# prashantpandeygit/solvingpapers

Hardware: AMD Instinct MI355X
Metric: training tokens/sec, LLaMA3-8B-shape bf16 (higher is better)
Workload: dtype bf16; 1 GPU; model=llama3_8b, global_batch=4, seq_len=8192, parallelism=dp1, micro_batch=1, grad_accum=4, params=8030261248

## Files before the change

csrc/include/attn_params.h:

```cpp
#pragma once
#include "attn_common.h"

#define SPA_DBG_BRH(b, r, R, h, H) (SPA_DBG_OK(b, p.B) & SPA_DBG_OK(r, R) & SPA_DBG_OK(h, H))

namespace spa {

struct AttnParams {
  const bf16* q; const bf16* k; const bf16* v; const bf16* o; const bf16* dout;
  bf16* out; bf16* dq; bf16* dk; bf16* dv;
  float* lse; const float* lse_in; float* delta; float* dqacc;
  int B, H, Hkv, Tq, Tk;
  long sqb, sqt, sqh, skb, skt, skh, svb, svt, svh, sob, sot, soh;
  long sdob, sdot, sdoh;
  long sdqb, sdqt, sdqh, sdkb, sdkt, sdkh, sdvb, sdvt, sdvh;
  float scale;
  float scale_log2;
  int causal_off;
  int hsplit;
  float* dkacc; float* dvacc;
  unsigned seed_lo, seed_hi, drop_thr;
  float drop_scale;
  const int64_t* seed_ptr;
  long long* stamp;
  int xcd;
  bf16* dsbuf;
  long ds_kvstride;
  int ds_nqt, ds_nkt;
  int ksplit;
  float* part;
  float* mlpart;
  int part_ld;
  int vhalf;
  float* rowk;
  int rowk_ld;
};

void launch_dkdv5(AttnParams& p, bool causal, hipStream_t st);
void launch_bwd_short(AttnParams& p, bool causal, hipStream_t st);

__device__ __forceinline__ long ds_index(int qt, int kt, int g, int G, int nkt, bool causal) {
  const int qb = qt >> 1, t = qt & 1;
  const long step = causal ? (long)qb * (qb + 1) + kt : (long)qb * nkt + kt;
  return (step * G + g) * 2 + t;
}
inline long ds_kv_elems(int nq64, int nkt, int G, bool causal) {
  return 1024L * 2 * G * (causal ? (long)nq64 * (nq64 + 1) : (long)nq64 * nkt);
}
__device__ __forceinline__ int ds_slot(int s, int h, int k) { return (k >> 2) * 16 + (2 * s + h) * 4 + (k & 3); }

template <int HD, int NDT = HD / 32>
__device__ __forceinline__ void store_kv_grad(const AttnParams& p, const f32x16 (&acc)[NDT], bool is_k,
                                              int b, int hk, int key, int split, int hh, int dt0 = 0) {
  if (key >= p.Tk) return;
  if (!(SPA_DBG_BRH(b, key, p.Tk, hk, p.Hkv) & SPA_DBG_OK(split, p.hsplit))) return;
  static_assert(NDT <= HD / 32, "store_kv_grad: more tiles than the head dim");
  constexpr int DT = NDT;
  if (p.hsplit == 1) {
    bf16* dst = (is_k ? p.dk + b * p.sdkb + (long)key * p.sdkt + hk * p.sdkh
                      : p.dv + b * p.sdvb + (long)key * p.sdvt + hk * p.sdvh) + 32 * dt0;
    const float sc = is_k ? p.scale : 1.f;
#pragma unroll
    for (int dt = 0; dt < DT; ++dt)
#pragma unroll
      for (int g = 0; g < 4; ++g) {
        bf16x4 w;
#pragma unroll
        for (int i = 0; i < 4; ++i) w[i] = (bf16)(acc[dt][4 * g + i] * sc);
        *reinterpret_cast<bf16x4*>(dst + 32 * dt + 8 * g + 4 * hh) = w;
      }
  } else {
    float* dst = (is_k ? p.dkacc : p.dvacc) +
                 ((((long)split * p.B + b) * p.Tk + key) * p.Hkv + hk) * HD + 32 * dt0;
#pragma unroll
    for (int dt = 0; dt < DT; ++dt)
#pragma unroll
      for (int g = 0; g < 4; ++g) {
        f32x4 w;
#pragma unroll
        for (int i = 0; i < 4; ++i) w[i] = acc[dt][4 * g + i];
        *reinterpret_cast<f32x4*>(dst + 32 * dt + 8 * g + 4 * hh) = w;
      }
  }
}


}
```

csrc/kernels/attention.hip:

```cpp
#include "attn_common.h"
#include "attn_params.h"

SPA_DEBUG_TU("attention.hip")

namespace spa {



__device__ __forceinline__ unsigned mix32(unsigned x) {
  x ^= x >> 16; x *= 0x7feb352dU; x ^= x >> 15; x *= 0x846ca68bU; x ^= x >> 16;
  return x;
}
__device__ __forceinline__ unsigned drop_base(const AttnParams& p, int b, int h) {
  unsigned lo = p.seed_lo, hi = p.seed_hi;
  if (p.seed_ptr) {
    const uint64_t sd = (uint64_t)*p.seed_ptr;
    lo = (unsigned)(sd & 0xffffffffu);
    hi = (unsigned)(sd >> 32);
  }
  return mix32(lo ^ mix32(hi + (unsigned)(b * p.H + h) * 0x9E3779B9U));
}
__device__ __forceinline__ bool drop_keep(unsigned base, int q, int key, unsigned thr) {
  return (mix32(base + (unsigned)q * 0x85EBCA6BU + (unsigned)key * 0xC2B2AE35U) >> 8) >= thr;
}
// ... 1258 lines not shown
      dso[ab] = 8 * ds_slot(g, pp & 1, key) + 4 * (pp >> 1);
    }
  }
  f32x16 acc[2][DT];
#pragma unroll
  for (int t = 0; t < 2; ++t)
#pragma unroll
    for (int i = 0; i < DT; ++i) acc[t][i] = splat16(0.f);

  auto compute = [&](int j, const bf16* sl) {
    if (j >= nsteps_w) return;
    const bf16* Ks = sl;
    const bf16* Dw = sl + KIMG + wave * WSLOT;
    const bool l0 = live(2 * qb, j), l1 = live(2 * qb + 1, j);
#pragma unroll
    for (int s = 0; s < 2; ++s) {
      bf16x8 kt[DT];
#pragma unroll
      for (int dt = 0; dt < DT; ++dt) kt[dt] = ld_tr(Ks + 16 * s * HD, off.tra[dt], off.trb[dt]);
      const bf16x8 d0 = ld_tr(Dw + 512 * s, dso[0], dso[1]);
      const bf16x8 d1 = ld_tr(Dw + 1024 + 512 * s, dso[0], dso[1]);
      if (l0) {
#pragma unroll
        for (int dt = 0; dt < DT; ++dt) acc[0][dt] = mfma32(kt[dt], d0, acc[0][dt]);
      }
      if (l1) {
#pragma unroll
        for (int dt = 0; dt < DT; ++dt) acc[1][dt] = mfma32(kt[dt], d1, acc[1][dt]);
      }
    }
  };
  if (nsteps > 0) issue(0, 0);
  if (nsteps > 1) issue(1, 1);
  for (int j = 0; j < nsteps; j += 3) {
#pragma unroll
    for (int r = 0; r < 3; ++r) {
      const int jj = j + r;
      if (jj < nsteps) {
        if (jj + 1 < nsteps) asm volatile("s_waitcnt vmcnt(6)" ::: "memory");
        else asm volatile("s_waitcnt vmcnt(0)" ::: "memory");
        asm volatile("s_waitcnt lgkmcnt(0)" ::: "memory");
        __builtin_amdgcn_s_barrier();
        if (jj + 2 < nsteps) issue(jj + 2, (r + 2) % 3);
        compute(jj, smem + r * SLOT);
      }
    }
  }
  if (!uvalid) return;
#pragma unroll
  for (int t = 0; t < 2; ++t) {
    const int q = qb * 64 + 32 * t + (lane & 31);
    if (q >= p.Tq || !SPA_DBG_BRH(b, q, p.Tq, h, p.H)) continue;
    bf16* op = p.dq + b * p.sdqb + (long)q * p.sdqt + h * p.sdqh;
#pragma unroll
    for (int dt = 0; dt < DT; ++dt)
#pragma unroll
      for (int g = 0; g < 4; ++g) {
        bf16x4 wv;
#pragma unroll
        for (int i = 0; i < 4; ++i) wv[i] = (bf16)(acc[t][dt][4 * g + i] * p.scale);
        *reinterpret_cast<bf16x4*>(op + 32 * dt + 8 * g + 4 * hh) = wv;
      }
  }
}

template <int HDK, bool CAUSAL, bool NT>
__global__ __launch_bounds__(256, 2) void attn_bwd_dq_ds256_kernel(AttnParams p) {
  static_assert(HDK == 256 || HDK == 192, "dq_ds256: q/k head dim 192 or 256");
  constexpr int HD = 256, DT = HDK / 32, KIMG = 32 * HD, WSLOT = 1024, SLOT = KIMG + 4 * WSLOT, NSLOT = 3;
  __shared__ __attribute__((aligned(16))) bf16 smem[NSLOT * SLOT];
  const int tid = threadIdx.x, lane = tid & 63;
  const int wave = __builtin_amdgcn_readfirstlane(tid >> 6);
  const int hh = lane >> 5;
  const int G = p.H / p.Hkv;
  const int nqt = cdiv(p.Tq, 32);
  const int upkv = nqt * G;
  const int wgpkv = cdiv(upkv, 4);
  const int nbkv = p.B * p.Hkv;
  const int bkv = blockIdx.x % nbkv;
  const int w = CAUSAL ? wgpkv - 1 - (int)(blockIdx.x / nbkv) : (int)(blockIdx.x / nbkv);
  const int b = bkv / p.Hkv, hk = bkv % p.Hkv;
  SPA_DBG_CHECK(b, p.B);
  const int u = 4 * w + wave;
  const bool uvalid = u < upkv;
  const int qt = uvalid ? u / G : 0;
  const int h = hk * G + (uvalid ? u % G : 0);
  auto unit_steps = [&](int uu) {
    const int qtt = uu / G;
    return CAUSAL ? cdiv(min(p.Tk, qtt * 32 + 32 + p.causal_off), 32) : cdiv(p.Tk, 32);
  };
  const int nsteps_w = uvalid ? unit_steps(u) : 0;
  const int nsteps = unit_steps(min(4 * w + 3, upkv - 1));

  const bf16* kbase = p.k + b * p.skb + hk * p.skh;
  unsigned kvo[4];
#pragma unroll
  for (int j = 0; j < 4; ++j) {
    const int r = 8 * wave + 2 * j + (lane >> 5);
    kvo[j] = (unsigned)(((long)r * p.skt + 8 * ((lane & 31) ^ swz<HD>(r))) * 2);
  }
  const bf16* dskv = p.dsbuf + ((long)b * p.Hkv + hk) * p.ds_kvstride;
  const int g = h - hk * G;
  auto live = [&](int kt) { return uvalid && qt < p.ds_nqt && (!CAUSAL || kt <= qt); };
  auto issue = [&](int j, int slot) {
    bf16* sl = smem + slot * SLOT;
    const int key0 = 32 * j;
// ... 342 lines not shown
        }
      } else {
        if (causal) attn_fwd_kernel<HDK_, HDV_, NW, true, false><<<gx, NW * 64, 0, st>>>(p);
        else attn_fwd_kernel<HDK_, HDV_, NW, false, false><<<gx, NW * 64, 0, st>>>(p);
      }
    });
  }
  if (p.ksplit > 1) {
    const long n = (long)B * H * Tq * (HDV / 8);
    HDKV_SWITCH(HDK, HDV, { attn_fwd_merge_kernel<HDV_><<<(int)cdiv(n, 256L), 256, 0, st>>>(p); });
  }
  SPA_LAUNCH_CHECK();
  return {out, lse};
}

template <int HDK, int HDV, bool DROP>
static void launch_bwd(AttnParams& p, bool causal, bool fused, int dkdv_mode, int nkv, hipStream_t st,
                       const at::TensorOptions& bf16_opts) {
  constexpr int NW = dq_waves<HDK, HDV>();
  constexpr int MT = (HDK <= 128 && HDV <= 128) ? 2 : 1;
  constexpr bool PAIRED_OK = HDK == HDV && HDK <= 128 && !DROP;
  const int g2 = nkv * p.hsplit;
  if constexpr (HDK == HDV && HDK <= 128 && !DROP) {
    if (fused) {
      const long rows = (long)p.B * p.Tq * p.H;
      attn_delta_kernel<HDK><<<(int)cdiv(rows, 256 / (HDK / 8)), 256, 0, st>>>(p);
      if (causal) attn_bwd_dkdv_kernel<HDK, HDV, true, MT, true, false><<<g2, 256, 0, st>>>(p);
      else attn_bwd_dkdv_kernel<HDK, HDV, false, MT, true, false><<<g2, 256, 0, st>>>(p);
      const long n = rows * (HDK / 8);
      attn_dq_store_kernel<HDK><<<(int)std::min<long>((n + 255) / 256, 65536), 256, 0, st>>>(p);
      return;
    }
  }
  if constexpr (HDK == 128 && HDV == 128 && !DROP) {
    const char* de = getenv("SPA_ATTN_DQ_DS");
    const bool want = !(de && atoi(de) == 0);
    const long kv_bytes = 2 * ds_kv_elems(cdiv(p.Tq, 64), cdiv(p.Tk, 32), p.H / p.Hkv, causal);
    if (want && p.hsplit == 1 && p.Tk > 0 && dkdv_mode == 0 && (!causal || p.causal_off == 0) &&
        kv_bytes < 0x7fffffffL) {
      const long rows = (long)p.B * p.Tq * p.H;
      const char* v5e = getenv("SPA_ATTN_DKDV5");
      const bool v5 = !(v5e && atoi(v5e) == 0);
      if (!v5) attn_delta_kernel<HDK><<<(int)cdiv(rows, 256 / (HDK / 8)), 256, 0, st>>>(p);
      p.ds_nqt = cdiv(p.Tq, 32);
      p.ds_nkt = cdiv(p.Tk, 32);
      p.ds_kvstride = ds_kv_elems(cdiv(p.Tq, 64), p.ds_nkt, p.H / p.Hkv, causal);
      at::Tensor dsb = at::empty({(long)p.B * p.Hkv * p.ds_kvstride}, bf16_opts);
      p.dsbuf = (bf16*)dsb.data_ptr();
      at::Tensor rowk;
      if (v5) {
        p.rowk_ld = cdiv(p.Tq, 64) * 64;
        rowk = at::empty({(long)p.B * p.H * 2 * p.rowk_ld}, bf16_opts.dtype(at::kFloat));
        p.rowk = rowk.data_ptr<float>();
        launch_dkdv5(p, causal, st);
      } else if (causal) attn_bwd_dkdv3_kernel<HDK, HDV, true, true><<<nkv, 512, 0, st>>>(p);
      else attn_bwd_dkdv3_kernel<HDK, HDV, false, true><<<nkv, 512, 0, st>>>(p);
      const int G = p.H / p.Hkv;
      const int wg = cdiv(cdiv(p.Tq, 64) * G, 4) * p.B * p.Hkv;
      const char* ne = getenv("SPA_ATTN_DS_NT");
      const bool nt = !(ne && atoi(ne) == 0);
      if (nt) {
        if (causal) attn_bwd_dq_ds_kernel<HDK, true, true><<<wg, 256, 0, st>>>(p);
        else attn_bwd_dq_ds_kernel<HDK, false, true><<<wg, 256, 0, st>>>(p);
      } else {
        if (causal) attn_bwd_dq_ds_kernel<HDK, true, false><<<wg, 256, 0, st>>>(p);
        else attn_bwd_dq_ds_kernel<HDK, false, false><<<wg, 256, 0, st>>>(p);
      }
      return;
    }
  }
  if constexpr (((HDK == 256 && HDV == 256) || (HDK == 192 && HDV == 128)) && !DROP) {
    const char* de = getenv("SPA_ATTN_DQ_DS");
    const int dsm = de ? atoi(de) : 1;
    const bool want = dsm != 0;
    const int G = p.H / p.Hkv;
    const long kv_bytes = 2 * ds_kv_elems(cdiv(p.Tq, 64), cdiv(p.Tk, 32), G, causal);
    const int wg = cdiv(cdiv(p.Tq, 32) * G, 4) * p.B * p.Hkv;
    if (want && (wg >= 512 || dsm == 2) && p.Tk > 0 && dkdv_mode == 0 && (!causal || p.causal_off == 0) &&
        kv_bytes < 0x7fffffffL) {
      const long rows = (long)p.B * p.Tq * p.H;
      attn_delta_kernel<HDV><<<(int)cdiv(rows, 256 / (HDV / 8)), 256, 0, st>>>(p);
      p.ds_nqt = cdiv(p.Tq, 32);
      p.ds_nkt = cdiv(p.Tk, 32);
      p.ds_kvstride = ds_kv_elems(cdiv(p.Tq, 64), p.ds_nkt, G, causal);
      at::Tensor dsb = at::empty({(long)p.B * p.Hkv * p.ds_kvstride}, bf16_opts);
      p.dsbuf = (bf16*)dsb.data_ptr();
      const int g2 = nkv * p.hsplit;
      bool paired_mla = false, dvs = false;
      AttnParams pk = p;
      at::Tensor dkpart;
      if constexpr (HDK == 256 && HDV == 256) {
        const char* ve = getenv("SPA_ATTN_DKDV256");
        dvs = !(ve && atoi(ve) == 0) && G % p.hsplit == 0;
        if (dvs) {
          if (causal) attn_bwd_dkdv3_kernel<HDK, HDV, true, true, true><<<g2, 512, 0, st>>>(p);
          else attn_bwd_dkdv3_kernel<HDK, HDV, false, true, true><<<g2, 512, 0, st>>>(p);
          int hs2 = p.hsplit;
          while (nkv * hs2 < 1024 && hs2 < G) {
            int d = hs2 + 1;
            while (G % d) ++d;
            hs2 = d;
          }
          pk.hsplit = hs2;
          if (hs2 > 1) {
            dkpart = at::empty({(long)hs2 * p.B * p.Tk * p.Hkv * HDK}, bf16_opts.dtype(at::kFloat));
            pk.dkacc = dkpart.data_ptr<float>();
// ... 19 lines not shown
      if (nt) {
        if (causal) attn_bwd_dq_ds256_kernel<HDK, true, true><<<wg, 256, 0, st>>>(p);
        else attn_bwd_dq_ds256_kernel<HDK, false, true><<<wg, 256, 0, st>>>(p);
      } else {
        if (causal) attn_bwd_dq_ds256_kernel<HDK, true, false><<<wg, 256, 0, st>>>(p);
        else attn_bwd_dq_ds256_kernel<HDK, false, false><<<wg, 256, 0, st>>>(p);
      }
      const long kr = (long)p.B * p.Tk * p.Hkv;
      if ((dvs ? pk : p).hsplit > 1)
        attn_kv_reduce_kernel<HDK><<<(int)std::min<long>((kr * (HDK / 8) + 255) / 256, 65536), 256, 0, st>>>(dvs ? pk : p, 1);
      if (p.hsplit > 1)
        attn_kv_reduce_kernel<HDV><<<(int)std::min<long>((kr * (HDV / 8) + 255) / 256, 65536), 256, 0, st>>>(p, 0);
      return;
    }
  }
  const int grid = cdiv(p.Tq, 32 * NW) * p.H * p.B;
  p.ksplit = p.Tk > 0 ? attn_ksplit(grid, cdiv(p.Tk, attn_bn<HDK, HDV>())) : 1;
  at::Tensor dqpart;
  if (p.ksplit > 1) {
    dqpart = at::empty({(long)p.ksplit * p.B * p.Tq * p.H * HDK}, bf16_opts.dtype(at::kFloat));
    p.part = dqpart.data_ptr<float>();
    p.part_ld = HDK;
  }
  if (causal) attn_bwd_dq_kernel<HDK, HDV, NW, true, DROP><<<grid * p.ksplit, NW * 64, 0, st>>>(p);
  else attn_bwd_dq_kernel<HDK, HDV, NW, false, DROP><<<grid * p.ksplit, NW * 64, 0, st>>>(p);
  if (p.ksplit > 1) {
    const long n = (long)p.B * p.Tq * p.H * (HDK / 8);
    attn_dq_reduce_kernel<HDK><<<(int)cdiv(n, 256L), 256, 0, st>>>(p);
  }
  if (p.Tk == 0) return;
  const bool piped = PAIRED_OK && (dkdv_mode == 3 || (dkdv_mode == 0 && HDV == 128));
  if (piped) {
    if constexpr (PAIRED_OK) {
      if (causal) attn_bwd_dkdv3_kernel<HDK, HDV, true><<<g2, 512, 0, st>>>(p);
      else attn_bwd_dkdv3_kernel<HDK, HDV, false><<<g2, 512, 0, st>>>(p);
    }
  } else {
    if (causal) attn_bwd_dkdv_kernel<HDK, HDV, true, MT, false, DROP><<<g2, 256, 0, st>>>(p);
    else attn_bwd_dkdv_kernel<HDK, HDV, false, MT, false, DROP><<<g2, 256, 0, st>>>(p);
  }
  if (p.hsplit > 1) {
    const long rows = (long)p.B * p.Tk * p.Hkv;
    attn_kv_reduce_kernel<HDK><<<(int)std::min<long>((rows * (HDK / 8) + 255) / 256, 65536), 256, 0, st>>>(p, 1);
    attn_kv_reduce_kernel<HDV><<<(int)std::min<long>((rows * (HDV / 8) + 255) / 256, 65536), 256, 0, st>>>(p, 0);
  }
}

static at::Tensor& last_stamps() {
  static at::Tensor t;
  return t;
}
at::Tensor attn_bwd_stamps() { return last_stamps().defined() ? last_stamps().view({-1, 8}).clone() : at::Tensor(); }

void attn_bwd(const at::Tensor& dout, const at::Tensor& q, const at::Tensor& k, const at::Tensor& v,
              const at::Tensor& out, const at::Tensor& lse, const at::Tensor& dq, const at::Tensor& dk,
              const at::Tensor& dv, double scale, bool causal, double dropout_p, int64_t seed,
              const c10::optional<at::Tensor>& seed_t) {
  check_qkv(dout, "dout"); check_qkv(q, "q"); check_qkv(k, "k"); check_qkv(v, "v"); check_qkv(out, "out");
  check_qkv(dq, "dq"); check_qkv(dk, "dk"); check_qkv(dv, "dv");
  const int B = q.size(0), Tq = q.size(1), H = q.size(2), HDK = q.size(3), HDV = v.size(3);
  const int Tk = k.size(1), Hkv = k.size(2);
  TORCH_CHECK(lse.is_contiguous() && lse.numel() == (int64_t)B * H * Tq);
  TORCH_CHECK(dq.sizes() == q.sizes() && dk.sizes() == k.sizes() && dv.sizes() == v.sizes());
  TORCH_CHECK(dout.sizes() == out.sizes() && out.size(3) == HDV && out.size(2) == H && out.size(1) == Tq);
  const bool drop = dropout_p > 0.0;
  TORCH_CHECK(!drop || HDK == HDV, "attn: dropout needs equal q/k and v head dims");
  DeviceGuard g(q.device());
  auto delta = at::empty({B, H, Tq}, q.options().dtype(at::kFloat));
  AttnParams p{};
  p.q = (const bf16*)q.data_ptr(); p.k = (const bf16*)k.data_ptr(); p.v = (const bf16*)v.data_ptr();
  p.o = (const bf16*)out.data_ptr(); p.dout = (const bf16*)dout.data_ptr();
  p.dq = (bf16*)dq.data_ptr(); p.dk = (bf16*)dk.data_ptr(); p.dv = (bf16*)dv.data_ptr();
  p.lse_in = lse.data_ptr<float>(); p.delta = delta.data_ptr<float>();
  p.B = B; p.H = H; p.Hkv = Hkv; p.Tq = Tq; p.Tk = Tk;
  fill_strides(p, q, k, v);
  fill_dropout(p, dropout_p, seed, seed_t);
  p.sob = out.stride(0); p.sot = out.stride(1); p.soh = out.stride(2);
  p.sdob = dout.stride(0); p.sdot = dout.stride(1); p.sdoh = dout.stride(2);
  p.sdqb = dq.stride(0); p.sdqt = dq.stride(1); p.sdqh = dq.stride(2);
  p.sdkb = dk.stride(0); p.sdkt = dk.stride(1); p.sdkh = dk.stride(2);
  p.sdvb = dv.stride(0); p.sdvt = dv.stride(1); p.sdvh = dv.stride(2);
  p.scale = (float)scale; p.scale_log2 = (float)(scale * 1.4426950408889634);
  p.causal_off = Tk - Tq;
  p.xcd = xcd_order(B, Hkv);
  p.ksplit = 1;
  if (B * H == 0) return;
  auto st = stream();
  if (Tq == 0) { dk.zero_(); dv.zero_(); return; }
  static const bool want_fused = getenv("SPA_ATTN_BWD_FUSED") && atoi(getenv("SPA_ATTN_BWD_FUSED")) != 0;
  const bool fused = want_fused && Tk > 0 && HDK <= 128 && HDK == HDV && !drop;
  const char* sse = getenv("SPA_ATTN_SHORT");
  const bool want_short = !(sse && atoi(sse) == 0);
  if (want_short && !fused && !drop && HDK == 64 && HDV == 64 && H == Hkv && Tq <= 256 && Tk <= 256) {
    launch_bwd_short(p, causal, st);
    SPA_LAUNCH_CHECK();
    return;
  }
  at::Tensor dqacc;
  if (fused) {
    dqacc = at::zeros({B, Tq, H, HDK}, q.options().dtype(at::kFloat));
    p.dqacc = dqacc.data_ptr<float>();
  }
  const int dkdv_mode = getenv("SPA_ATTN_DKDV") ? atoi(getenv("SPA_ATTN_DKDV")) : 0;
  const int G = H / Hkv;
  const int nkv = cdiv(Tk, 128) * Hkv * B;
  int hsplit = 1;
  const char* kbe = getenv("SPA_ATTN_KVBLOCKS");
  const int kvblocks = kbe ? std::max(1, atoi(kbe)) : 512;
  if (!fused)
    while (nkv * hsplit < kvblocks && hsplit < G) {
      int d = hsplit + 1;
      while (G % d) ++d;
      hsplit = d;
    }
  const bool pairedk = HDK == HDV && HDK <= 128 && !drop && (dkdv_mode == 3 || (dkdv_mode == 0 && HDV == 128));
  if (!fused && !pairedk)
    while (nkv * hsplit < kvblocks && hsplit < 16 && cdiv(Tq, 32) / (2 * hsplit) >= 4) hsplit *= 2;
  p.hsplit = hsplit;
  static at::Tensor stamps;
  const char* se = getenv("SPA_ATTN_STAMP");
  if (se && atoi(se) != 0) {
    const long need = (long)nkv * hsplit * 8 * 8;
    if (!stamps.defined() || stamps.numel() < need || stamps.device() != q.device())
      stamps = at::zeros({need}, q.options().dtype(at::kLong));
    p.stamp = (long long*)stamps.data_ptr<int64_t>();
    last_stamps() = stamps.narrow(0, 0, need);
  }
  at::Tensor kvacc;
  if (hsplit > 1) {
    kvacc = at::empty({(long)hsplit * B * Tk * Hkv * (HDK + HDV)}, q.options().dtype(at::kFloat));
    p.dkacc = kvacc.data_ptr<float>();
    p.dvacc = p.dkacc + (long)hsplit * B * Tk * Hkv * HDK;
  }
  HDKV_SWITCH(HDK, HDV, {
    if (drop) {
      if constexpr (HDK_ == HDV_) launch_bwd<HDK_, HDV_, true>(p, causal, false, dkdv_mode, nkv, st, q.options());
    } else {
      launch_bwd<HDK_, HDV_, false>(p, causal, fused, dkdv_mode, nkv, st, q.options());
    }
  });
  SPA_LAUNCH_CHECK();
}

}

TORCH_LIBRARY_FRAGMENT(spa, m) {
  m.def("attn_fwd(Tensor q, Tensor k, Tensor v, float scale, bool causal, float dropout_p=0.0, int seed=0, "
        "Tensor? seed_t=None) -> Tensor[]");
  m.def("attn_bwd(Tensor dout, Tensor q, Tensor k, Tensor v, Tensor out, Tensor lse, Tensor(a!) dq, Tensor(b!) dk, "
        "Tensor(c!) dv, float scale, bool causal, float dropout_p=0.0, int seed=0, Tensor? seed_t=None) -> ()");
  m.def("attn_bwd_stamps() -> Tensor", &spa::attn_bwd_stamps);
}
TORCH_LIBRARY_IMPL(spa, CUDA, m) {
  m.impl("attn_fwd", &spa::attn_fwd);
  m.impl("attn_bwd", &spa::attn_bwd);
}
```

csrc/kernels/attention_dkdv5.hip:

```cpp
#include "attn_common.h"
#include "attn_params.h"

SPA_DEBUG_TU("attention_dkdv5.hip")

namespace spa {

__device__ __forceinline__ void dma4_asm(__amdgpu_buffer_rsrc_t rs, unsigned voff, unsigned lds) {
  unsigned keep;
  asm volatile("s_mov_b32 %0, m0\n\ts_mov_b32 m0, %3\n\ts_nop 0\n\tbuffer_load_dword %1, %2, 0 offen lds\n\ts_mov_b32 m0, %0"
               : "=&s"(keep) : "v"(voff), "s"(rs), "s"(lds) : "memory");
}

template <int HD>
__global__ __launch_bounds__(256) void attn_rowk_kernel(AttnParams p) {
  constexpr int TPR = HD / 8, RPB = 256 / TPR;
  const int Tqp = p.rowk_ld;
  const long row = (long)blockIdx.x * RPB + threadIdx.x / TPR;
  const int t = threadIdx.x % TPR;
  const long nrows = (long)p.B * Tqp * p.H;
  float acc = 0.f;
  long b = 0, q = 0, h = 0;
  if (row < nrows) {
    h = row % p.H;
    q = (row / p.H) % Tqp;
// ... 238 lines not shown
        f32x16 dp;
#pragma unroll
        for (int g = 0; g < 4; ++g) {
          const f32x4 v = *reinterpret_cast<const f32x4*>(rcP + 32 * t + 8 * g + 4 * hh);
#pragma unroll
          for (int i = 0; i < 4; ++i) dp[4 * g + i] = v[i];
        }
#pragma unroll
        for (int ks = 0; ks < KS; ++ks) dp = mfma32(ld_row(Dp + 32 * t * HD, off.row[ks]), xf[ks], dp);
        const bf16x8 pa = *reinterpret_cast<const bf16x8*>(pr + (t * 2 + 0) * 512);
        const bf16x8 pb = *reinterpret_cast<const bf16x8*>(pr + (t * 2 + 1) * 512);
        f32x16 ds;
#pragma unroll
        for (int r = 0; r < 8; ++r) {
          ds[r] = (float)pa[r] * dp[r];
          ds[8 + r] = (float)pb[r] * dp[8 + r];
        }
        const bf16x8 sa = pack_acc(ds, 0), sb = pack_acc(ds, 1);
        const int qt = qtp + t;
        if ((!CAUSAL || kt <= qt) && qt < p.ds_nqt && kt < p.ds_nkt) store_ds(sa, sb, qt, tP.g);
        __builtin_amdgcn_sched_barrier(0);
#pragma unroll
        for (int dt = 0; dt < DT; ++dt) {
          acc[dt] = mfma32(ld_tr(Qp + 32 * t * HD, off.tra[dt], off.trb[dt]), sa, acc[dt]);
          acc[dt] = mfma32(ld_tr(Qp + (32 * t + 16) * HD, off.tra[dt], off.trb[dt]), sb, acc[dt]);
        }
        __builtin_amdgcn_sched_barrier(0);
      }
    }
    prev_act = cur;
    tP = tC;
    tC = tN;
    D5_TICK(1);
    asm volatile("s_waitcnt vmcnt(0)" ::: "memory");
    D5_TICK(2);
    asm volatile("s_waitcnt lgkmcnt(0)" ::: "memory");
    __builtin_amdgcn_s_barrier();
    D5_TICK(3);
  };
  if (total == 0) {
  } else if (role == 0) {
    for (int k = 0; k <= total; k += 3) {
      interval(k, IC<0>{}, IC<0>{});
      interval(k + 1, IC<1>{}, IC<0>{});
      interval(k + 2, IC<2>{}, IC<0>{});
    }
  } else {
    for (int k = 0; k <= total; k += 3) {
      interval(k, IC<0>{}, IC<1>{});
      interval(k + 1, IC<1>{}, IC<1>{});
      interval(k + 2, IC<2>{}, IC<1>{});
    }
  }
  store_kv_grad<HD>(p, acc, role == 1, b, hk, key, 0, hh);
#if SPA_DKDV5_STAMP
  D5_TICK(4);
  if (p.stamp != nullptr && lane < 8) {
    long long v = 0;
#pragma unroll
    for (int i = 0; i < 5; ++i) v = lane == i ? seg[i] : v;
    v = lane == 5 ? (long long)(total + 1) : lane == 6 ? ts_ - t_start : v;
    p.stamp[((long)blockIdx.x * 8 + wave) * 8 + lane] = v;
  }
#endif
}

void launch_dkdv5(AttnParams& p, bool causal, hipStream_t st) {
  const long rows = (long)p.B * p.rowk_ld * p.H;
  attn_rowk_kernel<128><<<(int)cdiv(rows, 256 / 16), 256, 0, st>>>(p);
  const int nkv = cdiv(p.Tk, 128) * p.Hkv * p.B;
  if (causal) attn_bwd_dkdv5_kernel<true><<<nkv, 512, 0, st>>>(p);
  else attn_bwd_dkdv5_kernel<false><<<nkv, 512, 0, st>>>(p);
}

}
```

solvingpapers_amd/models/llama3.py:

```python
from __future__ import annotations

import math
from dataclasses import dataclass, field, replace
from typing import List, Optional

import torch
import torch.nn as nn

from ..infer.cache import new_kv_cache
from ..infer.graph import DecodeState, ExtendState
from ..infer.sampling import sample
from ..ops import attention_packed, embedding, linear, linear_cross_entropy, rms_norm, rope_packed_
from ..ops.linear import swiglu_mlp
from ..ops.attention import kv_cache_attend, kv_cache_write, rope_kv_cache_write_
from ..ops.layout import gather_rows
from ..ops.rope import RopeCache, apply_rope
from ..utils.grad import mark_ready


@dataclass
class LlamaConfig:
    vocab_size: int = 50257
    dim: int = 256
    n_layers: int = 2
    n_heads: int = 4
    n_kv_heads: int = 2
    ffn_hidden: int = 1024
    max_seq_len: int = 128
    norm_eps: float = 1e-6
    rope_theta: float = 10000.0
    gate: str = "w3"
    ref_freqs: bool = True
    init: str = "ref"
    tie_embeddings: bool = False
    batch_size: int = 16
    lr: float = 3e-4

    @property
    def head_dim(self):
        return self.dim // self.n_heads


PRESETS = {
    "llama3_ref": LlamaConfig(),
    "llama3_8b": LlamaConfig(vocab_size=128256, dim=4096, n_layers=32, n_heads=32, n_kv_heads=8, ffn_hidden=14336,
                             max_seq_len=8192, norm_eps=1e-5, rope_theta=500000.0, gate="w1", init="std",
                             ref_freqs=False, batch_size=1, lr=3e-4),
    "llama3_tiny": LlamaConfig(vocab_size=1024, dim=512, n_layers=2, n_heads=4, n_kv_heads=2, ffn_hidden=1536,
                               max_seq_len=256, norm_eps=1e-5, rope_theta=500000.0, gate="w1", init="std",
                               ref_freqs=False, batch_size=2),
}


def config(name: str, **kw) -> LlamaConfig:
    return replace(PRESETS[name], **kw)


class LlamaBlock(nn.Module):
    def __init__(self, c: LlamaConfig, **fk):
        super().__init__()
        hd = c.head_dim
        self.c = c
        self.cp_group = None
        self.attention_norm = nn.Parameter(torch.ones(c.dim, **fk))
        self.wqkv = nn.Parameter(torch.empty((c.n_heads + 2 * c.n_kv_heads) * hd, c.dim, **fk))
        self.wo = nn.Parameter(torch.empty(c.dim, c.n_heads * hd, **fk))
        self.ffn_norm = nn.Parameter(torch.ones(c.dim, **fk))
        self.w13 = nn.Parameter(torch.empty(2 * c.ffn_hidden, c.dim, **fk))
        self.w2 = nn.Parameter(torch.empty(c.dim, c.ffn_hidden, **fk))

    @torch.no_grad()
    def reset_parameters(self, gen=None):
        c = self.c
        if c.init == "ref":
            for w in (self.wqkv, self.wo, self.w13, self.w2):
                nn.init.normal_(w, 0.0, 1.0, generator=gen).div_(math.sqrt(w.shape[1]))
            nn.init.normal_(self.attention_norm, 0.0, 1.0, generator=gen)
            nn.init.normal_(self.ffn_norm, 0.0, 1.0, generator=gen)
        else:
            for w in (self.wqkv, self.wo, self.w13, self.w2):
                nn.init.normal_(w, 0.0, 0.02, generator=gen)
            nn.init.ones_(self.attention_norm)
            nn.init.ones_(self.ffn_norm)

    def attn(self, n1, kv_cache=None, pos=0):
        c = self.c
        B, T, _ = n1.shape
        hd = c.head_dim
        qkv = linear(n1, self.wqkv)
        if isinstance(pos, DecodeState):
            H, KV = c.n_heads, c.n_kv_heads
            x4 = qkv.view(B, T, H + 2 * KV, hd)
            cos, sin = RopeCache.get(pos.max_len, hd, c.rope_theta, qkv.device, c.ref_freqs)
            rope_kv_cache_write_(kv_cache, x4, cos, sin, pos.positions, pos.index, H, KV, 0, per_row=pos.per_row)
            o = kv_cache_attend(x4[:, :, :H], kv_cache, causal=True, kv_len=pos.kv_len, per_row=pos.per_row)
            return linear(o.reshape(B, T, H * hd), self.wo)
        if kv_cache is None and self.cp_group is not None:
            import torch.distributed as dist
            from ..parallel.context_parallel import context_parallel_attention
            H, KV = c.n_heads, c.n_kv_heads
            off = dist.get_rank(self.cp_group) * T
            qkv = rope_packed_(qkv, H + KV, c.rope_theta, off, head_dim=hd, ref_freqs=c.ref_freqs)
            x4 = qkv.view(B, T, H + 2 * KV, hd)
            o = context_parallel_attention(x4[:, :, :H], x4[:, :, H:H + KV], x4[:, :, H + KV:], self.cp_group)
        elif kv_cache is None:
            qkv = rope_packed_(qkv, c.n_heads + c.n_kv_heads, c.rope_theta, 0, head_dim=hd, ref_freqs=c.ref_freqs)
            o = attention_packed(qkv, c.n_heads, c.n_kv_heads, causal=True, head_dim=hd)
        else:
            qkv = qkv.view(B, T, c.n_heads + 2 * c.n_kv_heads, hd)
            q = apply_rope(qkv[:, :, :c.n_heads], c.rope_theta, pos, ref_freqs=c.ref_freqs)
            k = apply_rope(qkv[:, :, c.n_heads:c.n_heads + c.n_kv_heads], c.rope_theta, pos, ref_freqs=c.ref_freqs)
            v = qkv[:, :, c.n_heads + c.n_kv_heads:]
            kv_cache_write(kv_cache, k, v, pos)
            o = kv_cache_attend(q, kv_cache, pos + T, causal=True, fresh=(k, v) if pos == 0 else None)
        return linear(o.reshape(B, T, c.n_heads * hd), self.wo)

    def forward(self, res, delta, kv_cache=None, pos=0):
        c = self.c
        if res is None:
            n1 = rms_norm(delta, self.attention_norm, c.norm_eps)
            h = delta
        else:
            n1, h = rms_norm(delta, self.attention_norm, c.norm_eps, residual=res)
        a = self.attn(n1, kv_cache, pos)
        n2, h2 = rms_norm(a, self.ffn_norm, c.norm_eps, residual=h)
        return h2, swiglu_mlp(n2, self.w13, self.w2, "silu")


class Llama3(nn.Module):
    def __init__(self, c: LlamaConfig, device=None, dtype=torch.float32, seed: int = 0):
        super().__init__()
        self.c = c
        fk = dict(device=device, dtype=dtype)
        self.tok_embeddings = nn.Parameter(torch.empty(c.vocab_size, c.dim, **fk))
        self.layers = nn.ModuleList([LlamaBlock(c, **fk) for _ in range(c.n_layers)])
        self.norm_f = nn.Parameter(torch.ones(c.dim, **fk))
        self.output = None if c.tie_embeddings else nn.Parameter(torch.empty(c.vocab_size, c.dim, **fk))
        self.grad_ready_cb = None
        self.param_wait_cb = None
        self.reset_parameters(seed)

    @torch.no_grad()
    def reset_parameters(self, seed=0):
        dev = self.tok_embeddings.device
        g = torch.Generator(device=dev).manual_seed(seed)
        c = self.c
        if c.init == "ref":
            nn.init.normal_(self.tok_embeddings, 0.0, 1.0, generator=g).div_(math.sqrt(c.vocab_size))
            nn.init.normal_(self.norm_f, 0.0, 1.0, generator=g)
            if self.output is not None:
                nn.init.normal_(self.output, 0.0, 1.0, generator=g).div_(math.sqrt(c.dim))
        else:
            nn.init.normal_(self.tok_embeddings, 0.0, 0.02, generator=g)
            nn.init.ones_(self.norm_f)
            if self.output is not None:
                nn.init.normal_(self.output, 0.0, 0.02, generator=g)
        for blk in self.layers:
            blk.reset_parameters(g)

    def param_groups(self) -> List[List[nn.Parameter]]:
# ... 122 lines not shown
```

solvingpapers_amd/ops/__init__.py:

```python
from . import _ext, reference
from .activation import act, elu, geglu, gelu, glu, leaky_relu, prelu, relu, sigmoid, silu, swiglu
from .attention import (KV8, attention_packed, decode_attention, flash_attention, kv_cache_attend, kv_cache_write,
                        rope_kv_cache_write_)
from .embedding import embedding
from .linear import Linear, linear
from .moe import MoEPlan, combine, gather, grouped_gemm, grouped_linear, moe_ffn, permute, route
from .norm import layer_norm, rms_norm
from .rope import apply_rope, rope_packed_
from .sampling import sample_logits, u01
from .xent import cross_entropy, linear_cross_entropy, per_row_loss

__all__ = [
    "act", "elu", "geglu", "gelu", "glu", "leaky_relu", "prelu", "relu", "sigmoid", "silu", "swiglu",
    "KV8", "kv_cache_attend", "kv_cache_write", "rope_kv_cache_write_",
    "attention_packed", "decode_attention", "flash_attention", "embedding", "Linear", "linear", "layer_norm", "rms_norm",
    "apply_rope", "rope_packed_", "MoEPlan", "combine", "gather", "grouped_gemm", "grouped_linear", "moe_ffn",
    "permute", "route", "cross_entropy", "linear_cross_entropy", "per_row_loss", "reference", "sample_logits", "u01",
]
```

solvingpapers_amd/ops/attention.py:

```python
from __future__ import annotations

import math

import os

import torch

from . import _ext, reference

FLASH_PAIRS = ((64, 64), (128, 128), (256, 256), (192, 128))
FLASH_HD = (64, 128, 256)


def _pair_for(dqk, dv):
    best = None
    for a, b in FLASH_PAIRS:
        if a >= dqk and b >= dv and (best is None or a + b < best[0] + best[1]):
            best = (a, b)
    return best


def _flash_ok(q):
    return q.is_cuda and q.dtype == torch.bfloat16 and (q.dim() == 3 or q.shape[-1] in FLASH_HD)

# ... 203 lines not shown
        dkr = dk[..., dn:].sum(2, keepdim=True, dtype=torch.float32).to(q.dtype)
        ops.rope_(dkr, cos, sin, None, 1, pos_off, 0, True)
        ops.rope_(dq[..., dn:], cos, sin, None, H, pos_off, 0, True)
        return dq, dkv, dkr, None, None, None, None


def mla_attention(q_raw, kv, kr, dn, scale, theta, pos_off=0):
    dr = q_raw.shape[-1] - dn
    dv = kv.shape[-1] - dn
    if (q_raw.is_cuda and q_raw.dtype == torch.bfloat16 and (dn + dr, dv) in ((192, 128), (128, 128))
            and kv.stride(-1) == 1 and kr.shape[2] == 1 and os.environ.get("SPA_MLA_FUSED", "1") != "0"):
        return _MLAFn.apply(q_raw, kv, kr, int(dn), float(scale), int(pos_off), float(theta))
    from .rope import apply_rope
    B, T, H, _ = q_raw.shape
    qr = apply_rope(q_raw[..., dn:], theta, pos_off)
    krr = apply_rope(kr, theta, pos_off)
    qf = torch.cat([q_raw[..., :dn], qr], dim=-1)
    k = torch.cat([kv[..., :dn], krr.expand(B, T, H, dr)], dim=-1)
    return flash_attention(qf, k, kv[..., dn:], causal=True, scale=scale)


class _SplitLastFn(torch.autograd.Function):

    @staticmethod
    def forward(ctx, x, a):
        ctx.a, ctx.shape = a, x.shape
        return x[..., :a].contiguous(), x[..., a:].contiguous()

    @staticmethod
    def backward(ctx, ga, gb):
        if ga is None:
            ga = torch.zeros(ctx.shape[:-1] + (ctx.a,), device=gb.device, dtype=gb.dtype)
        if gb is None:
            gb = torch.zeros(ctx.shape[:-1] + (ctx.shape[-1] - ctx.a,), device=ga.device, dtype=ga.dtype)
        return torch.cat([ga, gb], dim=-1), None


def split_last(x, a):
    return _SplitLastFn.apply(x, int(a))


def attention_packed(qkv, H, Hkv, causal=True, scale=None, head_dim=None, dropout_p=0.0, seed=None):
    hd = head_dim if head_dim is not None else qkv.shape[-1]
    B, T = qkv.shape[0], qkv.shape[1]
    scale = float(scale) if scale is not None else 1.0 / math.sqrt(hd)
    if dropout_p > 0.0 and seed is None:
        seed = torch.randint(0, 2 ** 62, (1,), device=qkv.device, dtype=torch.int64) if qkv.is_cuda else _new_seed()
    if qkv.is_cuda and qkv.dtype == torch.bfloat16 and hd in FLASH_HD:
        return _PackedFn.apply(qkv, H, Hkv, hd, causal, scale, float(dropout_p),
                               seed if isinstance(seed, torch.Tensor) else int(seed or 0))
    x4 = qkv.view(B, T, H + 2 * Hkv, hd)
    q, k, v = x4[:, :, :H], x4[:, :, H:H + Hkv], x4[:, :, H + Hkv:]
    return flash_attention(q, k, v, causal, scale, dropout_p, seed).reshape(B, T, H * hd)


class _PrefixPackedFn(torch.autograd.Function):

    @staticmethod
    def forward(ctx, qkv, qkv_a, H, Hkv, hd, scale):
        B, Tb, Ta = qkv.shape[0], qkv.shape[1], qkv_a.shape[1]
        c = H * hd
        kv = torch.cat([qkv_a[..., c:], qkv[..., c:]], dim=1)
        q4 = qkv.view(B, Tb, H + 2 * Hkv, hd)[:, :, :H]
        kv4 = kv.view(B, Ta + Tb, 2 * Hkv, hd)
        out, lse = _ext.ops().attn_fwd(q4, kv4[:, :, :Hkv], kv4[:, :, Hkv:], scale, True, 0.0, 0, None)
        ctx.save_for_backward(qkv, kv, out, lse)
        ctx.H, ctx.Hkv, ctx.hd, ctx.scale, ctx.Ta, ctx.shape_a = H, Hkv, hd, scale, Ta, qkv_a.shape
        return torch.ops.aten._unsafe_view(out, (B, Tb, H * hd))

    @staticmethod
    def backward(ctx, dout):
        qkv, kv, out, lse = ctx.saved_tensors
        H, Hkv, hd, Ta = ctx.H, ctx.Hkv, ctx.hd, ctx.Ta
        B, Tb = qkv.shape[0], qkv.shape[1]
        c = H * hd
        dqkv = torch.empty_like(qkv)
        dkv = torch.empty_like(kv)
        kv4, dkv4 = kv.view(B, Ta + Tb, 2 * Hkv, hd), dkv.view(B, Ta + Tb, 2 * Hkv, hd)
        _ext.ops().attn_bwd(dout.contiguous().view(B, Tb, H, hd), qkv.view(B, Tb, H + 2 * Hkv, hd)[:, :, :H],
                            kv4[:, :, :Hkv], kv4[:, :, Hkv:], out, lse,
                            dqkv.view(B, Tb, H + 2 * Hkv, hd)[:, :, :H], dkv4[:, :, :Hkv], dkv4[:, :, Hkv:],
                            ctx.scale, True, 0.0, 0, None)
        dqkv[..., c:] = dkv[:, Ta:]
        dqkv_a = torch.zeros(ctx.shape_a, device=dqkv.device, dtype=dqkv.dtype)
        dqkv_a[..., c:] = dkv[:, :Ta]
        return dqkv, dqkv_a, None, None, None, None


def attention_packed_prefix(qkv, qkv_a, H, Hkv, head_dim, scale=None):
    hd = head_dim
    B, Tb, Ta = qkv.shape[0], qkv.shape[1], qkv_a.shape[1]
    scale = float(scale) if scale is not None else 1.0 / math.sqrt(hd)
    if qkv.is_cuda and qkv.dtype == torch.bfloat16 and hd in FLASH_HD:
        return _PrefixPackedFn.apply(qkv, qkv_a, H, Hkv, hd, scale)
    xa, xb = qkv_a.view(B, Ta, H + 2 * Hkv, hd), qkv.view(B, Tb, H + 2 * Hkv, hd)
    k = torch.cat([xa[:, :, H:H + Hkv], xb[:, :, H:H + Hkv]], 1)
    v = torch.cat([xa[:, :, H + Hkv:], xb[:, :, H + Hkv:]], 1)
    return flash_attention(xb[:, :, :H], k, v, True, scale).reshape(B, Tb, H * hd)


def attention_dropout(q, k, v, causal=True, scale=None, p=0.0, training=True, neg=float("-inf")):
    if not training or p == 0.0:
        return flash_attention(q, k, v, causal, scale)
    scale = float(scale) if scale is not None else 1.0 / math.sqrt(q.shape[-1])
    if q.is_cuda:
        return flash_attention(q, k, v, causal, scale, dropout_p=p)
# ... 240 lines not shown
```

Baseline: 22540 tokens/s.

## Fold inverse RoPE into attention backward dQ/dK stores

Adds a fused rope+attention autograd function whose backward applies the inverse rotary embedding to dQ and dK inside the attention backward kernels' epilogues, instead of running a separate rope pass over the gradient. This removes one read-modify-write pass over the packed qkv gradient per layer. In exchange it adds cos/sin table loads in the store epilogue, and the non-folded fallback path still runs the separate rope kernel. Folding only applies for head dim 128, Tq==Tk, no dropout, and the dkdv5 path.

```diff
diff --git a/csrc/include/attn_params.h b/csrc/include/attn_params.h
--- a/csrc/include/attn_params.h
+++ b/csrc/include/attn_params.h
@@ -33,7 +33,35 @@
   int vhalf;
   float* rowk;
   int rowk_ld;
+  const float* rope_cos; const float* rope_sin;
+  int rope_off, rope_mode, rope_fold;
 };
+
+__device__ __forceinline__ f32x4 rope_inv_quad(const f32x16 (&acc)[4], int dt, int g, int hh, float sc,
+                                               const float* __restrict__ cr, const float* __restrict__ sr,
+                                               int mode) {
+  const int d0 = 32 * dt + 8 * g + 4 * hh;
+  f32x4 x, w;
+#pragma unroll
+  for (int i = 0; i < 4; ++i) x[i] = acc[dt][4 * g + i] * sc;
+  if (mode == 0) {
+    const float2 c = *reinterpret_cast<const float2*>(cr + (d0 >> 1));
+    const float2 s = *reinterpret_cast<const float2*>(sr + (d0 >> 1));
+    w[0] = x[0] * c.x + x[1] * s.x;
+    w[1] = x[1] * c.x - x[0] * s.x;
+    w[2] = x[2] * c.y + x[3] * s.y;
+    w[3] = x[3] * c.y - x[2] * s.y;
+  } else {
+    const f32x4 c = *reinterpret_cast<const f32x4*>(cr + (d0 & 63));
+    const f32x4 s = *reinterpret_cast<const f32x4*>(sr + (d0 & 63));
+#pragma unroll
+    for (int i = 0; i < 4; ++i) {
+      const float o = acc[dt ^ 2][4 * g + i] * sc;
+      w[i] = dt < 2 ? x[i] * c[i] + o * s[i] : x[i] * c[i] - o * s[i];
+    }
+  }
+  return w;
+}
 
 void launch_dkdv5(AttnParams& p, bool causal, hipStream_t st);
 void launch_bwd_short(AttnParams& p, bool causal, hipStream_t st);
@@ -48,13 +76,32 @@
 }
 __device__ __forceinline__ int ds_slot(int s, int h, int k) { return (k >> 2) * 16 + (2 * s + h) * 4 + (k & 3); }
 
-template <int HD, int NDT = HD / 32>
+template <int HD, int NDT = HD / 32, bool ROPE = false>
 __device__ __forceinline__ void store_kv_grad(const AttnParams& p, const f32x16 (&acc)[NDT], bool is_k,
                                               int b, int hk, int key, int split, int hh, int dt0 = 0) {
   if (key >= p.Tk) return;
   if (!(SPA_DBG_BRH(b, key, p.Tk, hk, p.Hkv) & SPA_DBG_OK(split, p.hsplit))) return;
   static_assert(NDT <= HD / 32, "store_kv_grad: more tiles than the head dim");
+  static_assert(!ROPE || (HD == 128 && NDT == 4), "store_kv_grad: the fold needs the whole hd-128 row");
   constexpr int DT = NDT;
+  if constexpr (ROPE) {
+    if (is_k && p.rope_fold) {
+      bf16* dst = p.dk + b * p.sdkb + (long)key * p.sdkt + hk * p.sdkh;
+      const float* cr = p.rope_cos + (long)(p.rope_off + key) * (HD / 2);
+      const float* sr = p.rope_sin + (long)(p.rope_off + key) * (HD / 2);
+#pragma unroll
+      for (int dt = 0; dt < DT; ++dt)
+#pragma unroll
+        for (int g = 0; g < 4; ++g) {
+          const f32x4 r = rope_inv_quad(acc, dt, g, hh, p.scale, cr, sr, p.rope_mode);
+          bf16x4 w;
+#pragma unroll
+          for (int i = 0; i < 4; ++i) w[i] = (bf16)r[i];
+          *reinterpret_cast<bf16x4*>(dst + 32 * dt + 8 * g + 4 * hh) = w;
+        }
+      return;
+    }
+  }
   if (p.hsplit == 1) {
     bf16* dst = (is_k ? p.dk + b * p.sdkb + (long)key * p.sdkt + hk * p.sdkh
                       : p.dv + b * p.sdvb + (long)key * p.sdvt + hk * p.sdvh) + 32 * dt0;
diff --git a/csrc/kernels/attention.hip b/csrc/kernels/attention.hip
--- a/csrc/kernels/attention.hip
+++ b/csrc/kernels/attention.hip
@@ -1334,6 +1334,21 @@
     const int q = qb * 64 + 32 * t + (lane & 31);
     if (q >= p.Tq || !SPA_DBG_BRH(b, q, p.Tq, h, p.H)) continue;
     bf16* op = p.dq + b * p.sdqb + (long)q * p.sdqt + h * p.sdqh;
+    if (p.rope_fold) {
+      const float* cr = p.rope_cos + (long)(p.rope_off + q) * (HD / 2);
+      const float* sr = p.rope_sin + (long)(p.rope_off + q) * (HD / 2);
+#pragma unroll
+      for (int dt = 0; dt < DT; ++dt)
+#pragma unroll
+        for (int g = 0; g < 4; ++g) {
+          const f32x4 r = rope_inv_quad(acc[t], dt, g, hh, p.scale, cr, sr, p.rope_mode);
+          bf16x4 wv;
+#pragma unroll
+          for (int i = 0; i < 4; ++i) wv[i] = (bf16)r[i];
+          *reinterpret_cast<bf16x4*>(op + 32 * dt + 8 * g + 4 * hh) = wv;
+        }
+      continue;
+    }
 #pragma unroll
     for (int dt = 0; dt < DT; ++dt)
 #pragma unroll
@@ -1782,6 +1797,7 @@
         p.rowk_ld = cdiv(p.Tq, 64) * 64;
         rowk = at::empty({(long)p.B * p.H * 2 * p.rowk_ld}, bf16_opts.dtype(at::kFloat));
         p.rowk = rowk.data_ptr<float>();
+        p.rope_fold = p.rope_cos != nullptr;
         launch_dkdv5(p, causal, st);
       } else if (causal) attn_bwd_dkdv3_kernel<HDK, HDV, true, true><<<nkv, 512, 0, st>>>(p);
       else attn_bwd_dkdv3_kernel<HDK, HDV, false, true><<<nkv, 512, 0, st>>>(p);
@@ -1907,10 +1923,15 @@
 }
 at::Tensor attn_bwd_stamps() { return last_stamps().defined() ? last_stamps().view({-1, 8}).clone() : at::Tensor(); }
 
-void attn_bwd(const at::Tensor& dout, const at::Tensor& q, const at::Tensor& k, const at::Tensor& v,
-              const at::Tensor& out, const at::Tensor& lse, const at::Tensor& dq, const at::Tensor& dk,
-              const at::Tensor& dv, double scale, bool causal, double dropout_p, int64_t seed,
-              const c10::optional<at::Tensor>& seed_t) {
+struct RopeFoldArgs {
+  const at::Tensor& cos; const at::Tensor& sin;
+  int64_t pos_off, mode;
+};
+
+static bool attn_bwd_impl(const at::Tensor& dout, const at::Tensor& q, const at::Tensor& k, const at::Tensor& v,
+                          const at::Tensor& out, const at::Tensor& lse, const at::Tensor& dq, const at::Tensor& dk,
+                          const at::Tensor& dv, double scale, bool causal, double dropout_p, int64_t seed,
+                          const c10::optional<at::Tensor>& seed_t, const RopeFoldArgs* rope) {
   check_qkv(dout, "dout"); check_qkv(q, "q"); check_qkv(k, "k"); check_qkv(v, "v"); check_qkv(out, "out");
   check_qkv(dq, "dq"); check_qkv(dk, "dk"); check_qkv(dv, "dv");
   const int B = q.size(0), Tq = q.size(1), H = q.size(2), HDK = q.size(3), HDV = v.size(3);
@@ -1939,9 +1960,26 @@
   p.causal_off = Tk - Tq;
   p.xcd = xcd_order(B, Hkv);
   p.ksplit = 1;
-  if (B * H == 0) return;
+  if (B * H == 0) return false;
   auto st = stream();
-  if (Tq == 0) { dk.zero_(); dv.zero_(); return; }
+  if (Tq == 0) { dk.zero_(); dv.zero_(); return false; }
+  if (rope) {
+    const char* fe = getenv("SPA_ATTN_ROPE_FOLD");
+    const at::Tensor& c = rope->cos;
+    const at::Tensor& s = rope->sin;
+    TORCH_CHECK(c.is_cuda() && s.is_cuda() && c.device() == q.device() && s.device() == q.device() &&
+                    c.scalar_type() == at::kFloat && s.scalar_type() == at::kFloat && c.dim() == 2 &&
+                    c.is_contiguous() && s.is_contiguous() && c.sizes() == s.sizes() && c.size(1) == HDK / 2,
+                "attn_bwd_rope: cos / sin must be contiguous fp32 [Tmax, hd/2] tables on q's device");
+    TORCH_CHECK(rope->pos_off >= 0 && rope->pos_off + std::max(Tq, Tk) <= c.size(0), "attn_bwd_rope: table too short");
+    TORCH_CHECK(rope->mode >= 0 && rope->mode <= 2, "attn_bwd_rope: mode must be 0, 1 or 2");
+    if (!(fe && atoi(fe) == 0) && rope->mode != 2 && Tq == Tk && HDK == 128 && HDV == 128 && !drop) {
+      p.rope_cos = c.data_ptr<float>();
+      p.rope_sin = s.data_ptr<float>();
+      p.rope_off = (int)rope->pos_off;
+      p.rope_mode = (int)rope->mode;
+    }
+  }
   static const bool want_fused = getenv("SPA_ATTN_BWD_FUSED") && atoi(getenv("SPA_ATTN_BWD_FUSED")) != 0;
   const bool fused = want_fused && Tk > 0 && HDK <= 128 && HDK == HDV && !drop;
   const char* sse = getenv("SPA_ATTN_SHORT");
@@ -1949,7 +1987,7 @@
   if (want_short && !fused && !drop && HDK == 64 && HDV == 64 && H == Hkv && Tq <= 256 && Tk <= 256) {
     launch_bwd_short(p, causal, st);
     SPA_LAUNCH_CHECK();
-    return;
+    return false;
   }
   at::Tensor dqacc;
   if (fused) {
@@ -1995,11 +2033,30 @@
     }
   });
   SPA_LAUNCH_CHECK();
+  return p.rope_fold != 0;
+}
+
+void attn_bwd(const at::Tensor& dout, const at::Tensor& q, const at::Tensor& k, const at::Tensor& v,
+              const at::Tensor& out, const at::Tensor& lse, const at::Tensor& dq, const at::Tensor& dk,
+              const at::Tensor& dv, double scale, bool causal, double dropout_p, int64_t seed,
+              const c10::optional<at::Tensor>& seed_t) {
+  attn_bwd_impl(dout, q, k, v, out, lse, dq, dk, dv, scale, causal, dropout_p, seed, seed_t, nullptr);
+}
+
+bool attn_bwd_rope(const at::Tensor& dout, const at::Tensor& q, const at::Tensor& k, const at::Tensor& v,
+                   const at::Tensor& out, const at::Tensor& lse, const at::Tensor& dq, const at::Tensor& dk,
+                   const at::Tensor& dv, double scale, bool causal, const at::Tensor& cos, const at::Tensor& sin,
+                   int64_t pos_off, int64_t mode) {
+  const RopeFoldArgs rope{cos, sin, pos_off, mode};
+  return attn_bwd_impl(dout, q, k, v, out, lse, dq, dk, dv, scale, causal, 0.0, 0, c10::nullopt, &rope);
 }
 
 }
 
 TORCH_LIBRARY_FRAGMENT(spa, m) {
+  m.def("attn_bwd_rope(Tensor dout, Tensor q, Tensor k, Tensor v, Tensor out, Tensor lse, Tensor(a!) dq, "
+        "Tensor(b!) dk, Tensor(c!) dv, float scale, bool causal, Tensor cos, Tensor sin, int pos_off, int mode) "
+        "-> bool");
   m.def("attn_fwd(Tensor q, Tensor k, Tensor v, float scale, bool causal, float dropout_p=0.0, int seed=0, "
         "Tensor? seed_t=None) -> Tensor[]");
   m.def("attn_bwd(Tensor dout, Tensor q, Tensor k, Tensor v, Tensor out, Tensor lse, Tensor(a!) dq, Tensor(b!) dk, "
@@ -2009,4 +2066,5 @@
 TORCH_LIBRARY_IMPL(spa, CUDA, m) {
   m.impl("attn_fwd", &spa::attn_fwd);
   m.impl("attn_bwd", &spa::attn_bwd);
-}
+  m.impl("attn_bwd_rope", &spa::attn_bwd_rope);
+}
diff --git a/csrc/kernels/attention_dkdv5.hip b/csrc/kernels/attention_dkdv5.hip
--- a/csrc/kernels/attention_dkdv5.hip
+++ b/csrc/kernels/attention_dkdv5.hip
@@ -314,7 +314,7 @@
       interval(k + 2, IC<2>{}, IC<1>{});
     }
   }
-  store_kv_grad<HD>(p, acc, role == 1, b, hk, key, 0, hh);
+  store_kv_grad<HD, HD / 32, true>(p, acc, role == 1, b, hk, key, 0, hh);
 #if SPA_DKDV5_STAMP
   D5_TICK(4);
   if (p.stamp != nullptr && lane < 8) {
diff --git a/solvingpapers_amd/models/llama3.py b/solvingpapers_amd/models/llama3.py
--- a/solvingpapers_amd/models/llama3.py
+++ b/solvingpapers_amd/models/llama3.py
@@ -10,7 +10,7 @@
 from ..infer.cache import new_kv_cache
 from ..infer.graph import DecodeState, ExtendState
 from ..infer.sampling import sample
-from ..ops import attention_packed, embedding, linear, linear_cross_entropy, rms_norm, rope_packed_
+from ..ops import embedding, linear, linear_cross_entropy, rms_norm, rope_attention_packed, rope_packed_
 from ..ops.linear import swiglu_mlp
 from ..ops.attention import kv_cache_attend, kv_cache_write, rope_kv_cache_write_
 from ..ops.layout import gather_rows
@@ -104,8 +104,8 @@
             x4 = qkv.view(B, T, H + 2 * KV, hd)
             o = context_parallel_attention(x4[:, :, :H], x4[:, :, H:H + KV], x4[:, :, H + KV:], self.cp_group)
         elif kv_cache is None:
-            qkv = rope_packed_(qkv, c.n_heads + c.n_kv_heads, c.rope_theta, 0, head_dim=hd, ref_freqs=c.ref_freqs)
-            o = attention_packed(qkv, c.n_heads, c.n_kv_heads, causal=True, head_dim=hd)
+            o = rope_attention_packed(qkv, c.n_heads, c.n_kv_heads, c.rope_theta, 0, causal=True, head_dim=hd,
+                                      ref_freqs=c.ref_freqs)
         else:
             qkv = qkv.view(B, T, c.n_heads + 2 * c.n_kv_heads, hd)
             q = apply_rope(qkv[:, :, :c.n_heads], c.rope_theta, pos, ref_freqs=c.ref_freqs)
diff --git a/solvingpapers_amd/ops/__init__.py b/solvingpapers_amd/ops/__init__.py
--- a/solvingpapers_amd/ops/__init__.py
+++ b/solvingpapers_amd/ops/__init__.py
@@ -1,7 +1,7 @@
 from . import _ext, reference
 from .activation import act, elu, geglu, gelu, glu, leaky_relu, prelu, relu, sigmoid, silu, swiglu
 from .attention import (KV8, attention_packed, decode_attention, flash_attention, kv_cache_attend, kv_cache_write,
-                        rope_kv_cache_write_)
+                        rope_attention_packed, rope_kv_cache_write_)
 from .embedding import embedding
 from .linear import Linear, linear
 from .moe import MoEPlan, combine, gather, grouped_gemm, grouped_linear, moe_ffn, permute, route
@@ -13,7 +13,7 @@
 __all__ = [
     "act", "elu", "geglu", "gelu", "glu", "leaky_relu", "prelu", "relu", "sigmoid", "silu", "swiglu",
     "KV8", "kv_cache_attend", "kv_cache_write", "rope_kv_cache_write_",
-    "attention_packed", "decode_attention", "flash_attention", "embedding", "Linear", "linear", "layer_norm", "rms_norm",
+    "attention_packed", "rope_attention_packed", "decode_attention", "flash_attention", "embedding", "Linear", "linear", "layer_norm", "rms_norm",
     "apply_rope", "rope_packed_", "MoEPlan", "combine", "gather", "grouped_gemm", "grouped_linear", "moe_ffn",
     "permute", "route", "cross_entropy", "linear_cross_entropy", "per_row_loss", "reference", "sample_logits", "u01",
 ]
diff --git a/solvingpapers_amd/ops/attention.py b/solvingpapers_amd/ops/attention.py
--- a/solvingpapers_amd/ops/attention.py
+++ b/solvingpapers_amd/ops/attention.py
@@ -279,6 +279,62 @@
     x4 = qkv.view(B, T, H + 2 * Hkv, hd)
     q, k, v = x4[:, :, :H], x4[:, :, H:H + Hkv], x4[:, :, H + Hkv:]
     return flash_attention(q, k, v, causal, scale, dropout_p, seed).reshape(B, T, H * hd)
+
+
+class _RopePackedFn(torch.autograd.Function):
+
+    @staticmethod
+    def forward(ctx, qkv, H, Hkv, hd, causal, scale, cos, sin, pos_off, mode):
+        B, T = qkv.shape[0], qkv.shape[1]
+        x4 = qkv.view(B, T, H + 2 * Hkv, hd)
+        ops = _ext.ops()
+        ops.rope_(x4, cos, sin, None, H + Hkv, pos_off, mode, False)
+        ctx.mark_dirty(qkv)
+        out, lse = ops.attn_fwd(x4[:, :, :H], x4[:, :, H:H + Hkv], x4[:, :, H + Hkv:], scale, causal, 0.0, 0, None)
+        ctx.save_for_backward(qkv, out, lse, cos, sin)
+        ctx.args = (H, Hkv, hd, causal, scale, pos_off, mode)
+        ctx.set_materialize_grads(False)
+        return qkv, torch.ops.aten._unsafe_view(out, (B, T, H * hd))
+
+    @staticmethod
+    def backward(ctx, dqkv_out, dout):
+        qkv, out, lse, cos, sin = ctx.saved_tensors
+        H, Hkv, hd, causal, scale, pos_off, mode = ctx.args
+        B, T = qkv.shape[0], qkv.shape[1]
+        ops = _ext.ops()
+        dqkv = torch.empty_like(qkv)
+        d4 = dqkv.view(B, T, H + 2 * Hkv, hd)
+        if dout is None:
+            dqkv.zero_()
+            folded = True
+        else:
+            x4 = qkv.view(B, T, H + 2 * Hkv, hd)
+            folded = ops.attn_bwd_rope(dout.contiguous().view(B, T, H, hd), x4[:, :, :H], x4[:, :, H:H + Hkv],
+                                       x4[:, :, H + Hkv:], out, lse, d4[:, :, :H], d4[:, :, H:H + Hkv],
+                                       d4[:, :, H + Hkv:], scale, causal, cos, sin, pos_off, mode)
+        if dqkv_out is not None:
+            if folded:
+                g = dqkv_out.contiguous().clone()
+                ops.rope_(g.view(B, T, H + 2 * Hkv, hd), cos, sin, None, H + Hkv, pos_off, mode, True)
+                dqkv.add_(g)
+            else:
+                dqkv.add_(dqkv_out)
+        if not folded:
+            ops.rope_(d4, cos, sin, None, H + Hkv, pos_off, mode, True)
+        return dqkv, None, None, None, None, None, None, None, None, None
+
+
+def rope_attention_packed(qkv, H, Hkv, theta=10000.0, pos_off=0, interleaved=True, causal=True, scale=None,
+                          head_dim=None, ref_freqs=False):
+    from .rope import RopeCache, _mode, rope_packed_
+    hd = head_dim if head_dim is not None else qkv.shape[-1]
+    if qkv.is_cuda and qkv.dtype == torch.bfloat16 and hd == 128 and interleaved in (True, False):
+        B, T = qkv.shape[0], qkv.shape[1]
+        scale = float(scale) if scale is not None else 1.0 / math.sqrt(hd)
+        cos, sin = RopeCache.get(pos_off + T, hd, theta, qkv.device, ref_freqs)
+        return _RopePackedFn.apply(qkv, H, Hkv, hd, causal, scale, cos, sin, int(pos_off), _mode(interleaved))[1]
+    qkv = rope_packed_(qkv, H + Hkv, theta, pos_off, interleaved, head_dim=head_dim, ref_freqs=ref_freqs)
+    return attention_packed(qkv, H, Hkv, causal=causal, scale=scale, head_dim=head_dim)
 
 
 class _PrefixPackedFn(torch.autograd.Function):
```

Result: no change. 22580 tokens/s (median of 6 runs) (+0.2%).
